# ruchikachavhan/diffusion-models-moe

Hardware: AMD Instinct MI355X
Metric: images/sec SD-1.4 512² 50-step DDIM, expert mask on; 1→8 GPU scaling (higher is better)
Workload: dtype fp16; 1 GPU; SD-1.4 MoE-fied (relu, top-k 0.2, expert 20) + RemoveExperts skilled-expert mask, 512^2 (4x64x64 latents), 50 DDIM steps, CFG 7.5; prompts_per_gpu=8, global_batch=8, parallelism=dp1

## Files before the change

diffusion-models-moe_amd/csrc/gemm.hip:

```cpp
#include <array>
#include <utility>

#include "tune.h"
#include "../../include/sdmoe.h"
#include "gemm_kernel.h"

namespace {

enum TileId { T128x160, T64x160, T256x320, T256x160_42, T256x320_42, T128x320, T128x160_42, T64x320, T128x32, T128x64,
              T128x128, T64x128, NTILE };
struct TileShape { int bm, bn, wmw, wnw; };
constexpr TileShape kTile[NTILE] = {{128, 160, 2, 2}, {64, 160, 2, 2}, {256, 320, 2, 4}, {256, 160, 4, 2},
                                    {256, 320, 4, 2}, {128, 320, 2, 4}, {128, 160, 4, 2}, {64, 320, 2, 4},
                                    {128, 32, 2, 2},  {128, 64, 2, 2},  {128, 128, 2, 2}, {64, 128, 2, 2}};
struct Plan {
  int mode;
  int tile;
  int bk, stages;
  int ksplit;
  int kchunk;
  int kchunk2;
  int mfast;
};
struct TileRule { int tile, ks_want, stages_want; };

constexpr bool built(int mode, int tile) {
  if (mode_halo(mode)) return (tile == T128x320 && mode != MODE_CONVHUP64) || (tile == T256x320 && mode != MODE_CONVHUP16);
  if (mode_geglu(mode))
    return tile == T128x160 || tile == T64x160 || tile == T256x320 || tile == T256x160_42 || tile == T256x320_42 ||
           (tile == T128x160_42 && mode != MODE_GEGLU_GT);
  if (tile == T128x160_42 || tile == T64x320) return mode == MODE_GEMM || mode == MODE_CONV || mode == MODE_GEMM_LN;
  if (tile == T128x32) return mode == MODE_CONV;
  return true;
}
constexpr bool fits3(const TileShape& t, int mode) {
  return GemmLayout{t.bm, t.bn, t.wmw, t.wnw, mode, 3, 64}.SMEM <= 160 * 1024;
}

int device_cus() {
  static int cus = 0;
  int dev = 0, n = 0;
  if (!cus && hipGetDevice(&dev) == hipSuccess &&
// ... 22 lines not shown
    if (ksplit > nk / 4) ksplit = nk / 4;
  }
  while (ksplit > 1 && (long)ksplit * p.M * p.N > ws_floats) --ksplit;
  if (ksplit < 1) ksplit = 1;
  const int kchunk = (nk + ksplit - 1) / ksplit;
  return (nk + kchunk - 1) / kchunk;
}

Plan tile_plan(int mode, int tile, const GemmParams& p, int ksplit, int stages_want) {
  const TileShape& t = kTile[tile];
  const int ntiles = ((p.M + t.bm - 1) / t.bm) * ((p.N + t.bn - 1) / t.bn);
  const int nk = p.K / 64;
  Plan pl{};
  pl.mode = mode; pl.tile = tile; pl.bk = 64; pl.ksplit = ksplit;
  pl.kchunk = (nk + ksplit - 1) / ksplit;
  pl.mfast = (pl.ksplit > 1 && knob(KNOB_MFAST) && (mode == MODE_CONV || mode == MODE_CONV_UP)) ? 1 : 0;
  const int stages = knob(KNOB_STAGES) ? knob(KNOB_STAGES)
                                       : (stages_want ? stages_want : ((t.wmw * t.wnw == 4 && ntiles * pl.ksplit >= 300) ? 2 : 3));
  pl.stages = (stages == 2 || !fits3(t, mode)) ? 2 : 3;
  return pl;
}


Plan halo_plan(int tile, int mode, const GemmParams& p, bool ws, long ws_floats) {
  const int cus = device_cus();
  const int ntiles = (p.M / kTile[tile].bm) * (p.N / 320);
  const int nsl = p.Cin / 32;
  int ksplit = 1;
  const int forced = knob(KNOB_KSPLIT);
  if (ws && forced > 0) {
    ksplit = forced < nsl ? forced : nsl;
// ... 145 lines not shown
  return plan_launch(p.upsample ? MODE_CONV_UP : MODE_CONV, p, ws, ws_floats);
}

template <int MODE, int TILE>
int launch_kernel(const Plan& pl, const GemmParams& p, dim3 grid, hipStream_t s) {
  constexpr TileShape t = kTile[TILE];
  constexpr int NTH = 64 * t.wmw * t.wnw;
  if constexpr (!built(MODE, TILE)) return SDMOE_EUNSUP;
  else if constexpr (mode_halo(MODE)) gemm_kernel<t.bm, t.bn, t.wmw, t.wnw, MODE, 4, 32><<<grid, NTH, 0, s>>>(p);
  else if constexpr (!fits3(t, MODE)) gemm_kernel<t.bm, t.bn, t.wmw, t.wnw, MODE, 2, 64><<<grid, NTH, 0, s>>>(p);
  else if (pl.stages == 2) gemm_kernel<t.bm, t.bn, t.wmw, t.wnw, MODE, 2, 64><<<grid, NTH, 0, s>>>(p);
  else gemm_kernel<t.bm, t.bn, t.wmw, t.wnw, MODE, 3, 64><<<grid, NTH, 0, s>>>(p);
  return SDMOE_OK;
}

constexpr int NMODE = MODE_GEGLU_GT + 1;
using LaunchFn = int (*)(const Plan&, const GemmParams&, dim3, hipStream_t);
template <int... KEY>
constexpr std::array<LaunchFn, sizeof...(KEY)> launch_table(std::integer_sequence<int, KEY...>) {
  return {{&launch_kernel<KEY / NTILE, KEY % NTILE>...}};
}
constexpr auto kLaunch = launch_table(std::make_integer_sequence<int, NMODE * NTILE>{});

int launch(const Plan& pl, GemmParams p, float* ws, hipStream_t s) {
  const TileShape& t = kTile[pl.tile];
  if (p.w_bstride && p.rows_per_batch % t.bm) return SDMOE_EUNSUP;
  if (p.image_set && p.rows_per_batch % t.bm) return SDMOE_EUNSUP;
  if (pl.ksplit > 1 && !ws) return SDMOE_EARG;
  p.ksplit = pl.ksplit; p.kchunk = pl.kchunk; p.kchunk2 = pl.kchunk2; p.mfast = pl.mfast;
  p.part = pl.ksplit > 1 ? ws : nullptr;
  p.diag = knob(KNOB_DIAG); p.res16 = knob(KNOB_RES16);
  const int direct = knob(KNOB_EPI_DIRECT);
  p.epi_direct = direct == 2 || (direct == 1 && p.R == nullptr);
  const dim3 grid(((p.M + t.bm - 1) / t.bm) * ((p.N + t.bn - 1) / t.bn) * pl.ksplit);
  if (const int st = kLaunch[pl.mode * NTILE + pl.tile](pl, p, grid, s)) return st;
  SDMOE_CHECK_LAUNCH();
  if (pl.ksplit > 1) {
    long nchunk = (long)p.M * (p.N / 8);
    int g = (int)((nchunk + 255) / 256);
    if (g > 2048) g = 2048;
    splitk_reduce_kernel<<<g, 256, 0, s>>>(p);
    SDMOE_CHECK_LAUNCH();
  }
  return SDMOE_OK;
}



__global__ __launch_bounds__(256) void gn_apply_kernel(const half_t* __restrict__ X, long ldx, int HW, int C,
                                                       const float* __restrict__ scale, const float* __restrict__ shift,
                                                       int silu, half_t* __restrict__ Y, long ldy, long rows) {
  const int cpr = C / 8;
  const long n = rows * cpr;
  for (long id = blockIdx.x * 256L + threadIdx.x; id < n; id += (long)gridDim.x * 256) {
    const long r = id / cpr;
    const int c = (int)(id - r * cpr) * 8;
// ... 397 lines not shown

extern "C" int sdmoe_conv3x3(const void* X, long ldx, int nimg, int H, int W, int Cin,
                             const void* Wt, const void* bias, const void* coladd, long coladd_bstride,
                             const void* R, long ldr, void* Y, long ldy, int Cout, int stride, int upsample,
                             int act, float* workspace, long workspace_floats, void* stream) {
  if (nimg == 0) return SDMOE_OK;
  if (!X || !Wt || !Y || nimg < 0 || H <= 0 || W <= 0 || Cout <= 0) return SDMOE_EARG;
  if (Cin % 64 || Cout % 8 || ldx % 8 || ldy % 8 || (R && ldr % 8)) return SDMOE_ESHAPE;
  if (!(stride == 1 || stride == 2) || (upsample && stride != 1)) return SDMOE_EUNSUP;
  GemmParams p{};
  conv_shape(p, nimg, H, W, Cin, 0, Cout, stride, upsample, act);
  if (const int st = fill_conv(p, X, ldx, Wt, bias, coladd, coladd_bstride, R, ldr, nullptr, 0, Y, ldy)) return st;
  return launch(plan_conv(p, workspace, workspace_floats), p, workspace, (hipStream_t)stream);
}

extern "C" int sdmoe_conv3x3_sc(const void* X, long ldx, int nimg, int H, int W, int Cin, const void* Wt,
                                const void* bias, const void* coladd, long coladd_bstride, const void* X2, long ldx2,
                                int Cin2, void* Y, long ldy, int Cout, int act, float* workspace,
                                long workspace_floats, void* stream) {
  if (nimg == 0) return SDMOE_OK;
  if (!X || !Wt || !X2 || !Y || nimg < 0 || H <= 0 || W <= 0 || Cout <= 0 || Cin2 <= 0) return SDMOE_EARG;
  if (Cin % 64 || Cin2 % 64 || Cout % 8 || ldx % 8 || ldx2 % 8 || ldy % 8) return SDMOE_ESHAPE;
  GemmParams p{};
  conv_shape(p, nimg, H, W, Cin, Cin2, Cout, 1, 0, act);
  if (const int st = fill_conv(p, X, ldx, Wt, bias, coladd, coladd_bstride, nullptr, 0, X2, ldx2, Y, ldy)) return st;
  return launch(plan_conv(p, workspace, workspace_floats), p, workspace, (hipStream_t)stream);
}

extern "C" int sdmoe_conv3x3_gn(const void* X, long ldx, int nimg, int H, int W, int Cin, const float* gn_scale,
                                const float* gn_shift, int silu, const void* Wt, const void* bias, const void* coladd,
// ... 46 lines not shown
```

diffusion-models-moe_amd/csrc/gemm_kernel.h:

```cpp
#pragma once
#include <type_traits>
#include <utility>
#include "common.h"

namespace {

typedef __attribute__((address_space(3))) void lds_void_t;

struct GemmParams {
  const half_t* A; long lda;
  const half_t* W; long ldw;
  const half_t* bias;
  const half_t* coladd; long coladd_bstride;
  const half_t* R; long ldr;
  half_t* C; long ldc;
  float* part;
  int M, N, K;
  int act;
  int rows_per_batch;
  int H, Wd, Cin, OH, OW, stride, upsample;
  int ksplit, kchunk;
  int kchunk2;
  int mfast;
  int a_bytes, w_bytes;
// ... 78 lines not shown
      for (int j = 0; j < 8; ++j) v[j] += (float)rr[j];
    }
  }
  half8 o;
#pragma unroll
  for (int j = 0; j < 8; ++j) o[j] = (half_t)v[j];
  if (p.diag & 8) {
    asm volatile("" ::"v"(o));
    return;
  }
  *reinterpret_cast<half8*>(p.C + (long)m * p.ldc + n) = o;
}

enum { MODE_GEMM = 0, MODE_CONV = 1, MODE_CONV_UP = 2, MODE_GEGLU = 3, MODE_KEEP = 4, MODE_WMASK = 5, MODE_KEEPW = 6,
       MODE_GEMM_LN = 7, MODE_GEGLU_LN = 8, MODE_CONVH64 = 9, MODE_CONVH32 = 10, MODE_CONVH16 = 11,
       MODE_CONVHUP64 = 12, MODE_CONVHUP32 = 13, MODE_CONVHUP16 = 14, MODE_GEGLU_GT = 15 };
constexpr bool mode_halo(int mode) { return mode >= MODE_CONVH64 && mode <= MODE_CONVHUP16; }
constexpr bool mode_halo_up(int mode) { return mode >= MODE_CONVHUP64 && mode <= MODE_CONVHUP16; }
constexpr int halo_w(int mode) {
  return (mode == MODE_CONVH64 || mode == MODE_CONVHUP64) ? 64 : ((mode == MODE_CONVH32 || mode == MODE_CONVHUP32) ? 32 : 16);
}
constexpr bool mode_akeep(int mode) { return mode == MODE_KEEP || mode == MODE_KEEPW; }
constexpr bool mode_wmask(int mode) { return mode == MODE_WMASK || mode == MODE_KEEPW; }
constexpr bool mode_geglu(int mode) { return mode == MODE_GEGLU || mode == MODE_GEGLU_LN || mode == MODE_GEGLU_GT; }
constexpr bool mode_ln(int mode) { return mode == MODE_GEMM_LN || mode == MODE_GEGLU_LN; }

constexpr int keep_a_bytes(int bm, int mode) { return mode_akeep(mode) ? ((bm * 8 + 1023) / 1024) * 1024 : 0; }
constexpr int keep_w_bytes(int bn, int mode) { return mode_wmask(mode) ? ((bn * 8 + 1023) / 1024) * 1024 : 0; }
constexpr int keep_stage_bytes(int bm, int bn, int mode) { return keep_a_bytes(bm, mode) + keep_w_bytes(bn, mode); }
constexpr int keep_lut_bytes(int mode) { return mode == MODE_KEEP ? 256 * 16 : 16 * 8; }

// ... 30 lines not shown
  int EPI = NW * (WM / NPASS) * WN_PAD * 4, EPI16 = NW * (WM / NPASS16) * RS16 * 2;
  int SMEM0 = (RINGX > EPI) ? (RINGX > EPI16 ? RINGX : EPI16) : (EPI > EPI16 ? EPI : EPI16);
  int LUT_OFF = SMEM0;
  int SMEM1 = SMEM0 + (keep ? keep_lut_bytes(mode) : 0);
  int LN_ROW_OFF = SMEM1, LN_COL_OFF = SMEM1 + bm * 8, LN_IPL = ln ? (bm * 8) / NT : 1;
  int SMEM = SMEM1 + (ln ? bm * 8 + bn * 8 : 0);
  int G_STAGING = NW * 2 * (16 * (FM % 2 == 0 ? 2 : 1)) * (WN / 2) * 2 + NW * WN * 4;
  bool TAB_PREFETCH = mode == MODE_GEGLU_GT && STAGE >= TAB_BYTES && G_STAGING <= STAGE;
  int TAB_LATE_OFF = ((G_STAGING + 1023) / 1024) * 1024;
  bool TAB_OK = mode == MODE_GEGLU_GT && (TAB_PREFETCH || TAB_LATE_OFF + TAB_BYTES <= SMEM1);
};

template <int BM_, int BN_, int WMW_, int WNW_, int MODE_, int NSTAGE_, int BKT_>
struct GemmCfg {
  static constexpr int BM = BM_, BN = BN_, WMW = WMW_, WNW = WNW_, MODE = MODE_, NSTAGE = NSTAGE_, BK = BKT_;
  static constexpr bool CONV = MODE == MODE_CONV || MODE == MODE_CONV_UP, GEGLU = mode_geglu(MODE), LN = mode_ln(MODE);
  static constexpr bool AKEEP = mode_akeep(MODE), WKEEP = mode_wmask(MODE), KEEP = AKEEP || WKEEP;
  static constexpr bool HALO = mode_halo(MODE), HUP = mode_halo_up(MODE);
  static constexpr GemmLayout lay() { return GemmLayout{BM, BN, WMW, WNW, MODE, NSTAGE, BK}; }
  static constexpr int swzk(int row) { return (row >> 1) & (BK / 8 - 1); }
};

SDMOE_DEV float add_f16_lo(float acc, unsigned x) {
  asm("v_fma_mix_f32 %0, %1, 1.0, %0 op_sel_hi:[1,0,0]" : "+v"(acc) : "v"(x));
  return acc;
}
SDMOE_DEV float add_f16_hi(float acc, unsigned x) {
  asm("v_fma_mix_f32 %0, %1, 1.0, %0 op_sel:[1,0,0] op_sel_hi:[1,0,0]" : "+v"(acc) : "v"(x));
  return acc;
}

// ... 49 lines not shown
    tm = bid % ntm;
    const int r = bid / ntm;
    tn = r % ntn;
    split = r / ntn;
  } else {
    split = bid % p.ksplit;
    const int tile = bid / p.ksplit;
    tn = tile % ntn;
    tm = tile / ntn;
  }
  const int m0 = tm * BM, n0 = tn * BN;
  const int nk_total = p.K / BK;
  const int ks0 = split * p.kchunk;
  const int ks1 = min(nk_total, ks0 + p.kchunk);
  const int nk = ks1 - ks0;

  const __amdgpu_buffer_rsrc_t rsA = __builtin_amdgcn_make_buffer_rsrc((void*)p.A, (short)0, p.a_bytes, 0x00020000);
  const half_t* Wimg = p.w_bstride ? p.W + (long)(m0 / p.rows_per_batch) * p.w_bstride : p.W;
  const __amdgpu_buffer_rsrc_t rsW = __builtin_amdgcn_make_buffer_rsrc((void*)Wimg, (short)0, p.w_bytes, 0x00020000);
  const int lrow = lane / L.CPRW, lch = lane % L.CPRW;
  unsigned avoff[L.A_PW];
  unsigned amask[L.A_PW];
  int aoh[L.A_PW], aow[L.A_PW], ab_[L.A_PW];
  unsigned avoff2[L.A_PW];
  unsigned bvoff[L.B_PW];
#pragma unroll
  for (int j = 0; j < L.A_PW; ++j) {
    const int r = L.RPP * (j * L.NW + wave) + lrow;
    const unsigned chb = (unsigned)((lch ^ G::swzk(r)) * 16);
    const int m = m0 + r;
// ... 4 lines not shown
        avoff[j] = (unsigned)((long)m * p.lda * 2) + chb;
      } else {
        const int hw = p.OH * p.OW;
        const int b = m / hw, rr = m - b * hw;
        const int oh = rr / p.OW, ow = rr - oh * p.OW;
        if (MODE == MODE_CONV) {
          const int ih = oh * p.stride, iw = ow * p.stride;
          avoff[j] = (unsigned)(((long)(b * p.H + ih) * p.Wd + iw) * p.lda * 2) + chb;
          unsigned msk = 0;
#pragma unroll
          for (int t = 0; t < 9; ++t) {
            const int y = ih + t / 3 - 1, x = iw + t % 3 - 1;
            msk |= (y >= 0 && y < p.H && x >= 0 && x < p.Wd) ? (1u << t) : 0u;
          }
          amask[j] = msk;
        } else {
          amask[j] = 1; avoff[j] = chb; aoh[j] = oh; aow[j] = ow; ab_[j] = b;
        }
      }
    }
  }
#pragma unroll
  for (int j = 0; j < L.B_PW; ++j) {
    const int r = L.RPP * (j * L.NW + wave) + lrow;
    const int n = n0 + r;
    bvoff[j] = (j * L.NW + wave < L.B_INS && n < p.N) ? (unsigned)((long)n * p.ldw * 2) + (unsigned)((lch ^ G::swzk(r)) * 16)
                                                  : OOB;
  }
  const int kpiece = G::KEEP && wave < L.K_INS ? wave : 0;
  const bool kpa = G::AKEEP && kpiece < L.KA_INS;
// ... 19 lines not shown
        *reinterpret_cast<uint4v*>(smem + L.LUT_OFF + e * 16) = m;
      }
    } else if (tid < 16) {
      const unsigned lo = ((tid & 1) ? 0xFFFFu : 0u) | ((tid & 2) ? 0xFFFF0000u : 0u);
      const unsigned hi = ((tid & 4) ? 0xFFFFu : 0u) | ((tid & 8) ? 0xFFFF0000u : 0u);
      *reinterpret_cast<uint2v*>(smem + L.LUT_OFF + tid * 8) = (uint2v){lo, hi};
    }
    __syncthreads();
  }
  auto a_dst = [&](int j) { return (j * L.NW + wave < L.A_INS) ? (j * L.NW + wave) * 1024 : L.STAGE_AB; };
  auto b_dst = [&](int j) { return (j * L.NW + wave < L.B_INS) ? BM * BK * 2 + (j * L.NW + wave) * 1024 : L.STAGE_AB; };

  const int csl = G::CONV ? p.Cin / BK : 0;
  const __amdgpu_buffer_rsrc_t rsA2 =
      __builtin_amdgcn_make_buffer_rsrc((void*)p.A2, (short)0, p.A2 ? p.a2_bytes : 0, 0x00020000);
  int st_c = G::CONV ? ks0 / 9 : 0, st_tap = G::CONV ? ks0 - st_c * 9 : 0;
  if (MODE == MODE_CONV && ks0 >= 9 * csl) { st_c = csl + (ks0 - 9 * csl); st_tap = 0; }

  auto issue_stage = [&](int ks, int buf) {
    char* sa = smem + buf * L.STAGE;
    const unsigned kb = (unsigned)(ks * BK * 2);
    if (p.diag & 16) {
    } else if (!G::CONV) {
#pragma unroll
      for (int j = 0; j < L.A_PW; ++j) bld16(rsA, sa + a_dst(j), avoff[j], kb);
    } else if (MODE == MODE_CONV && st_c >= csl) {
      const unsigned c2b = (unsigned)((st_c - csl) * BK * 2);
      ++st_c;
#pragma unroll
      for (int j = 0; j < L.A_PW; ++j) bld16(rsA2, sa + a_dst(j), avoff2[j] == OOB ? OOB : avoff2[j] + c2b, 0);
    } else {
      const int tap = st_tap;
      const int kh = tap >= 6 ? 2 : (tap >= 3 ? 1 : 0);
      const int kw = tap - 3 * kh;
      const int c0b = st_c * BK * 2;
      if (++st_tap == 9) { st_tap = 0; ++st_c; }
      if (MODE == MODE_CONV) {
        const unsigned tapoff = (unsigned)(((kh - 1) * p.Wd + (kw - 1)) * (int)p.lda * 2 + c0b);
#pragma unroll
        for (int j = 0; j < L.A_PW; ++j) {
          const unsigned vo = ((amask[j] >> tap) & 1u) ? avoff[j] + tapoff : OOB;
          bld16(rsA, sa + a_dst(j), vo, 0);
        }
      } else {
#pragma unroll
// ... 483 lines not shown
        const float rstd = rsqrtf(var + p.ln_eps);
        ln_row[2 * row] = rstd;
        ln_row[2 * row + 1] = -mean * rstd;
      }
    }
    for (int c = tid; c < BN; c += L.NT) {
      const bool ok = n0 + c < p.N;
      ln_col[c] = ok ? p.ln_wsum[n0 + c] : 0.f;
      ln_col[BN + c] = ok ? p.ln_bias[n0 + c] : 0.f;
    }
  }
  __syncthreads();
  constexpr int CPR = L.WN / 8;
  if (!G::GEGLU && p.act == ACT_NONE && (!p.R || p.res16 != 0)) {
    half4 b4[L.FN];
#pragma unroll
    for (int j = 0; j < L.FN; ++j) {
      const int n = nw + 16 * j + 4 * fg;
      b4[j] = (!G::LN && p.bias && n < p.N) ? *reinterpret_cast<const half4*>(p.bias + n) : (half4){0, 0, 0, 0};
    }
    if (!G::WKEEP && p.epi_direct) {
      const bool res = p.R != nullptr;
#pragma unroll
      for (int i = 0; i < L.FM; ++i) {
        __builtin_amdgcn_sched_barrier(0);
        const int m = mw + 16 * i + fr;
        const half_t* cap = (p.coladd && m < p.M) ? p.coladd + (long)(m / p.rows_per_batch) * p.coladd_bstride : nullptr;
        const float* cfp = (p.colf && m < p.M) ? p.colf + (long)(m / p.rows_per_batch) * p.colf_bstride : nullptr;
        float a = 0.f, c = 0.f;
        if constexpr (G::LN) {
          const int rl = wr * L.WM + 16 * i + fr;
          a = ln_row[2 * rl];
          c = ln_row[2 * rl + 1];
        }
// ... 26 lines not shown
        };
#pragma unroll
        for (int j = 0; j + 1 < L.FN; j += 2) {
          const uint2v ya = frag16(j), yb = frag16(j + 1);
          const auto s0 = __builtin_amdgcn_permlane16_swap(ya[0], yb[0], false, false);
          const auto s1 = __builtin_amdgcn_permlane16_swap(ya[1], yb[1], false, false);
          const int n = nw + 16 * (j + (fg & 1)) + 8 * (fg >> 1);
          half8 o = __builtin_bit_cast(half8, (uint4v){s0[0], s1[0], s0[1], s1[1]});
          if (m < p.M && n < p.N) {
            if (res) {
              const half8 rr = *reinterpret_cast<const half8*>(p.R + (long)m * p.ldr + n);
#pragma unroll
              for (int r = 0; r < 8; ++r) o[r] = (half_t)((float)o[r] + (float)rr[r]);
            }
            if (p.diag & 8) asm volatile("" ::"v"(o));
            else *reinterpret_cast<half8*>(p.C + (long)m * p.ldc + n) = o;
          }
        }
        if constexpr (L.FN % 2) {
          const int n = nw + 16 * (L.FN - 1) + 4 * fg;
          half4 o = __builtin_bit_cast(half4, frag16(L.FN - 1));
          if (m < p.M && n < p.N) {
            if (res) {
              const half4 rr = *reinterpret_cast<const half4*>(p.R + (long)m * p.ldr + n);
#pragma unroll
              for (int r = 0; r < 4; ++r) o[r] = (half_t)((float)o[r] + (float)rr[r]);
            }
            if (p.diag & 8) asm volatile("" ::"v"(o));
            else *reinterpret_cast<half4*>(p.C + (long)m * p.ldc + n) = o;
          }
        }
      }
      return;
    }
    half_t* st = reinterpret_cast<half_t*>(smem) + wave * (L.WM / L.NPASS16) * L.RS16;
    constexpr int NCH16 = (L.WM / L.NPASS16) * CPR, NIT16 = (NCH16 + 63) / 64;
    const bool res = p.R != nullptr;
#pragma unroll
    for (int h = 0; h < L.NPASS16; ++h) {
      half8 rr[NIT16];
      if (res) {
#pragma unroll
        for (int it = 0; it < NIT16; ++it) {
          const int id = lane + 64 * it;
// ... 45 lines not shown
        }
      }
      wave_sync();
#pragma unroll
      for (int it = 0; it < NIT16; ++it) {
        const int id = lane + 64 * it;
        const int r = id / CPR, c8 = id - r * CPR;
        const int m = mw + h * (L.WM / L.NPASS16) + r, n = nw + c8 * 8;
        if (id >= NCH16 || m >= p.M || n >= p.N) continue;
        half8 o = *reinterpret_cast<const half8*>(st + r * L.RS16 + c8 * 8);
        if (res) {
#pragma unroll
          for (int j = 0; j < 8; ++j) o[j] = (half_t)((float)o[j] + (float)rr[it][j]);
        }
        if (p.diag & 8) asm volatile("" ::"v"(o));
        else *reinterpret_cast<half8*>(p.C + (long)m * p.ldc + n) = o;
      }
      wave_sync();
    }
    return;
  }
  if constexpr (G::GEGLU) {
    int lane_o = lane;
    asm volatile("" : "+v"(lane_o));
    const int fr_e = lane_o & 15, fg_e = lane_o >> 4;
    typedef _Float16 h2 __attribute__((ext_vector_type(2)));
    constexpr int NH = L.WN / 2;
    constexpr int FPP = L.FM % 2 == 0 ? 2 : 1;
    constexpr int RG = 16 * FPP;
    constexpr int GST = L.NW * 2 * RG * NH * 2;
    static_assert(NH % 8 == 0, "whole 16-B product chunks per row");
    static_assert(GST + L.NW * L.WN * 4 <= L.SMEM1, "GEGLU staging and bias must fit in the kernel's LDS");
    static_assert(GST + L.NW * L.WN * 4 == L.G_STAGING, "GEGLU staging size as the layout states it");
    constexpr bool gtab = L.TAB_OK;
    char* const sbase = (L.TAB_PREFETCH && gtab) ? smem + ((nk - 1) % NSTAGE) * L.STAGE : smem;
    const half_t* const tab = reinterpret_cast<const half_t*>(
// ... 109 lines not shown
__global__ __launch_bounds__(256) void splitk_reduce_kernel(GemmParams p) {
  const long nchunk = (long)p.M * (p.N / 8);
  for (long id = blockIdx.x * 256L + threadIdx.x; id < nchunk; id += (long)gridDim.x * 256) {
    const int m = (int)(id / (p.N / 8)), n = (int)(id % (p.N / 8)) * 8;
    float v[8] = {0, 0, 0, 0, 0, 0, 0, 0};
    for (int s = 0; s < p.ksplit; ++s) {
      const float* sp = p.part + ((long)s * p.M + m) * p.N + n;
      float4v a = *reinterpret_cast<const float4v*>(sp), b = *reinterpret_cast<const float4v*>(sp + 4);
      v[0] += a[0]; v[1] += a[1]; v[2] += a[2]; v[3] += a[3];
      v[4] += b[0]; v[5] += b[1]; v[6] += b[2]; v[7] += b[3];
    }
    epilogue8(p, m, n, v);
  }
}

}
```

diffusion-models-moe_amd/sdmoe/_lib.py:

```python
from __future__ import annotations

import ctypes
import os

_HERE = os.path.dirname(os.path.abspath(__file__))
LIB_PATH = os.path.join(_HERE, "libsdmoe_hip.so")

_P = ctypes.c_void_p
_L = ctypes.c_long
_I = ctypes.c_int
_F = ctypes.c_float
_FP = ctypes.POINTER(ctypes.c_float)
_IP = ctypes.POINTER(ctypes.c_int)

SIGNATURES = {
    "sdmoe_linear": [_P, _L, _P, _L, _P, _P, _L, _I, _P, _L, _P, _L, _I, _I, _I, _I, _P, _L, _P],
    "sdmoe_conv3x3": [_P, _L, _I, _I, _I, _I, _P, _P, _P, _L, _P, _L, _P, _L, _I, _I, _I, _I, _P, _L, _P],
    "sdmoe_conv3x3_sc": [_P, _L, _I, _I, _I, _I, _P, _P, _P, _L, _P, _L, _I, _P, _L, _I, _I, _P, _L, _P],
    "sdmoe_conv3x3_gn": [_P, _L, _I, _I, _I, _I, _P, _P, _I, _P, _P, _P, _L, _P, _L, _P, _L, _I, _P, _L, _I, _P, _L,
                         _P],
    "sdmoe_groupnorm_apply": [_P, _L, _I, _I, _I, _P, _P, _I, _P, _L, _P],
    "sdmoe_mask_weight": [_P, _P, _L, _L, _P, _P],
    "sdmoe_groupnorm_stats": [_P, _L, _I, _I, _I, _I, _P, _P, _F, _P, _P, _P, _L, _P],
    "sdmoe_groupnorm": [_P, _L, _I, _I, _I, _I, _P, _P, _F, _I, _P, _L, _P, _P, _P, _L, _P],
    "sdmoe_gn_fold": [_P, _L, _I, _I, _P, _P, _P, _I, _P, _P, _P],
    "sdmoe_linear_per_image": [_P, _L, _P, _L, _L, _P, _L, _I, _P, _L, _P, _L, _I, _I, _I, _P, _L, _P],
    "sdmoe_layernorm": [_P, _L, _P, _L, _I, _I, _P, _P, _F, _P],
    "sdmoe_ln_fold": [_P, _L, _I, _I, _P, _P, _P, _P, _L, _P, _P, _P],
    "sdmoe_linear_ln": [_P, _L, _P, _L, _P, _P, _F, _P, _L, _I, _I, _I, _P],
    "sdmoe_linear_geglu_ln": [_P, _L, _P, _L, _P, _P, _F, _P, _L, _I, _I, _I, _I, _P, _L, _I, _P],
    "sdmoe_attention": [_P, _L, _P, _L, _P, _L, _P, _L, _I, _I, _I, _I, _I, _F, _P],
    "sdmoe_geglu_route": [_P, _L, _I, _I, _I, _I, _I, _P, _P, _P, _P, _P, _L, _P, _L, _P, _P, _P],
    "sdmoe_score_bias": [_P, _L, _I, _I, _P, _P, _L, _P],
    "sdmoe_geglu_route_bias": [_P, _L, _I, _I, _I, _I, _I, _P, _P, _P, _P, _P, _L, _P, _L, _P, _P, _P, _P],
    "sdmoe_linear_geglu": [_P, _L, _P, _L, _P, _P, _L, _I, _I, _I, _I, _P, _L, _I, _P],
# ... 112 lines not shown
```

diffusion-models-moe_amd/sdmoe/ops.py:

```python
from __future__ import annotations

import ctypes
import os

import torch

from . import _lib

ACT_NONE, ACT_SILU, ACT_GELU, ACT_RELU, ACT_QUICK_GELU = 0, 1, 2, 3, 4
ACT_BY_NAME = {"none": ACT_NONE, "silu": ACT_SILU, "gelu": ACT_GELU, "relu": ACT_RELU, "quick_gelu": ACT_QUICK_GELU}


_raw_stream = getattr(torch._C, "_cuda_getCurrentRawStream", None)
_cur_dev = getattr(torch._C, "_cuda_getDevice", None)


def _stream():
    if _raw_stream is not None and _cur_dev is not None:
        return _raw_stream(_cur_dev())
    return torch.cuda.current_stream().cuda_stream


def _ptr(t):
    return None if t is None else t.data_ptr()
# ... 362 lines not shown
def conv3x3_launch(xp, ldx, nimg, H, W, Cin, w, bias, coladd, coladd_bstride, rp, ldr, out, op, ldy, Cout, stride,
                   upsample, act, sc=None):
    lib = _lib.load()
    ws = _workspace(out.device)
    if sc is not None:
        st = lib.sdmoe_conv3x3_sc(xp, ldx, nimg, H, W, Cin, _dev(w, "w"), _ptr(bias), _ptr(coladd), coladd_bstride,
                                  sc[0], sc[1], sc[2], op, ldy, Cout, act, ws.data_ptr(), ws.numel(), _stream())
        _lib.check(st, "sdmoe_conv3x3_sc")
        return out
    st = lib.sdmoe_conv3x3(xp, ldx, nimg, H, W, Cin, _dev(w, "w"), _ptr(bias), _ptr(coladd), coladd_bstride, rp, ldr,
                           op, ldy, Cout, stride, int(bool(upsample)), act, ws.data_ptr(), ws.numel(), _stream())
    _lib.check(st, "sdmoe_conv3x3")
    return out


def groupnorm_stats(x, nimg, HW, gamma, beta, eps, groups=32):
    lib = _lib.load()
    xp, ldx = _rows(x, "x")
    C = x.shape[1]
    scale = torch.empty((nimg, C), dtype=torch.float32, device=x.device)
    shift = torch.empty((nimg, C), dtype=torch.float32, device=x.device)
    ws = _gn_workspace(x.device, nimg * groups * 64 * 2)
    st = lib.sdmoe_groupnorm_stats(xp, ldx, nimg, HW, C, groups, _dev(gamma, "gamma"), _dev(beta, "beta"),
                                   float(eps), scale.data_ptr(), shift.data_ptr(), ws.data_ptr(), ws.numel(),
                                   _stream())
    _lib.check(st, "sdmoe_groupnorm_stats")
    return scale, shift


def groupnorm(x, nimg, HW, gamma, beta, eps, groups=32, silu=False, out=None):
# ... 698 lines not shown
```

diffusion-models-moe_amd/sdmoe/unet.py:

```python
from __future__ import annotations

import os

import torch
import torch.nn as nn
import torch.nn.functional as F

from . import ops
from .config import UNetConfig

CTX_LEN = 77
FUSED_GEGLU = True
FUSED_KEEP = True
FUSED_LN = os.environ.get("SDMOE_FUSED_LN", "1") != "0"
FUSED_LN_FFN = os.environ.get("SDMOE_FUSED_LN_FFN", "0") == "1"
FUSED_SC = os.environ.get("SDMOE_FUSED_SC", "1") != "0"
FUSED_GN = os.environ.get("SDMOE_FUSED_GN", "1") != "0"
GN_FOLD_MIN_HW = 1024
IN_PAD = 64
OUT_PAD = 8


def _buf(t):
    return nn.Parameter(t, requires_grad=False)


class LoRACompatibleLinear(nn.Module):

    def __init__(self, weight, bias=None):
        super().__init__()
        self.weight = _buf(weight)
        self.bias = None if bias is None else _buf(bias)
        self._sdmoe_deferred = 0
# ... 428 lines not shown
        if ops.conv_gn_fusable(H, W, cmid, self.conv2.weight.shape[0]):
            gn2 = self.norm2.stats(h, nimg, HW) + (True,)
        else:
            hn = self.norm2.normalize(h, nimg, HW, True)
        if self.conv_shortcut is not None and FUSED_SC and x.shape[1] % 64 == 0:
            w, b = self._conv2_with_shortcut()
            return ops.conv3x3(hn, nimg, H, W, w, b, shortcut=x, out=out, gn=gn2)
        res = x if self.conv_shortcut is None else self.conv_shortcut.run(x)
        return ops.conv3x3(hn, nimg, H, W, self.conv2.weight, self.conv2.bias, residual=res, out=out, gn=gn2)


class Sampler(nn.Module):
    def __init__(self, conv):
        super().__init__()
        self.conv = conv


class Block(nn.Module):

    def __init__(self, resnets, attentions=None, downsamplers=None, upsamplers=None):
        super().__init__()
        self.resnets = nn.ModuleList(resnets)
        if attentions:
            self.attentions = nn.ModuleList(attentions)
        else:
            self.attentions = None
        if downsamplers:
            self.downsamplers = nn.ModuleList(downsamplers)
        if upsamplers:
            self.upsamplers = nn.ModuleList(upsamplers)
# ... 217 lines not shown
                has_up = hasattr(blk, "upsamplers")
                if not last_in_block:
                    nb, ncp, _ = up_in[idx + 1]
                    dest = nb[:, :ncp]
                elif has_up or i == nblk - 1:
                    dest = new(rows, cout)
                if blk.attentions is not None:
                    r = blk.resnets[j].run(inp, nimg, hh, hh, temb_all, out=new(rows, cout))
                    o = blk.attentions[j].run(r, nimg, hh * hh, ctx2d, out=dest)
                else:
                    o = blk.resnets[j].run(inp, nimg, hh, hh, temb_all, out=dest)
                idx += 1
                if last_in_block:
                    if has_up:
                        nb, ncp, _ = up_in[idx]
                        c = blk.upsamplers[0].conv
                        ops.conv3x3(o, nimg, hh, hh, c.weight, c.bias, upsample=True, out=nb[:, :ncp])
                    else:
                        final = o

        fn = self.conv_norm_out.normalize(final, nimg, H * W, True)
        if out is None:
            out = new(nimg * H * W, OUT_PAD)
        return ops.conv3x3(fn, nimg, H, W, self.conv_out.weight, self.conv_out.bias, out=out)

    def forward(self, sample, timestep, encoder_hidden_states, added_cond_kwargs=None):
        n, c, H, W = sample.shape
        x = torch.zeros((n * H * W, IN_PAD), dtype=torch.float16, device=sample.device)
        x[:, :c] = sample.permute(0, 2, 3, 1).reshape(n * H * W, c).to(torch.float16)
        ctx = encoder_hidden_states.reshape(-1, encoder_hidden_states.shape[-1]).to(torch.float16).contiguous()
        add_hidden = None
        if self.config.addition_embed_type == "text_time":
# ... 4 lines not shown
```

include/sdmoe.h:

```cpp
#ifndef SDMOE_H
#define SDMOE_H

#ifdef __cplusplus
extern "C" {
#endif

#define SDMOE_ACT_NONE 0
#define SDMOE_ACT_SILU 1
#define SDMOE_ACT_GELU 2
#define SDMOE_ACT_RELU 3
#define SDMOE_ACT_QUICK_GELU 4

const char* sdmoe_version(void);

int sdmoe_linear(const void* A, long lda, const void* W, long ldw, const void* bias, const void* coladd,
                 long coladd_bstride, int rows_per_batch, const void* R, long ldr, void* C, long ldc, int M, int N,
                 int K, int act, float* workspace, long workspace_floats, void* stream);

int sdmoe_conv3x3(const void* X, long ldx, int nimg, int H, int W, int Cin, const void* Wt, const void* bias,
                  const void* coladd, long coladd_bstride, const void* R, long ldr, void* Y, long ldy, int Cout,
                  int stride, int upsample, int act, float* workspace, long workspace_floats, void* stream);

int sdmoe_conv3x3_sc(const void* X, long ldx, int nimg, int H, int W, int Cin, const void* Wt, const void* bias,
                     const void* coladd, long coladd_bstride, const void* X2, long ldx2, int Cin2, void* Y, long ldy,
                     int Cout, int act, float* workspace, long workspace_floats, void* stream);

int sdmoe_conv3x3_gn(const void* X, long ldx, int nimg, int H, int W, int Cin, const float* gn_scale,
                     const float* gn_shift, int silu, const void* Wt, const void* bias, const void* coladd,
                     long coladd_bstride, const void* R, long ldr, const void* X2, long ldx2, int Cin2, void* Y,
                     long ldy, int Cout, float* workspace, long workspace_floats, void* stream);
int sdmoe_groupnorm_apply(const void* X, long ldx, int nimg, int HW, int C, const float* scale, const float* shift,
                          int silu, void* Y, long ldy, void* stream);

int sdmoe_mask_weight(const void* W, const void* bits, long N, long K, void* Wm, void* stream);

int sdmoe_groupnorm_stats(const void* X, long ldx, int nimg, int HW, int C, int groups, const void* gamma,
                          const void* beta, float eps, float* scale, float* shift, float* workspace,
                          long workspace_floats, void* stream);

int sdmoe_groupnorm(const void* X, long ldx, int nimg, int HW, int C, int groups, const void* gamma, const void* beta,
                    float eps, int silu, void* Y, long ldy, float* scale, float* shift, float* workspace,
                    long workspace_floats, void* stream);

int sdmoe_gn_fold(const void* W, long ldw, int N, int K, const void* bias, const float* scale, const float* shift,
                  int nimg, void* Wf, float* colbias, void* stream);
// ... 131 lines not shown
```

Baseline: 9.390 images/s.

## Collapse nearest-upsample 3x3 conv into four 2x2 sub-pixel convolutions

Adds an UP2X GEMM mode that folds nearest-neighbour 2x upsampling followed by a 3x3 conv into four phase-specific 2x2 convs. The weights are pre-collapsed and cached, and the epilogue and split-K reduce scatter results to interleaved output pixels. This cuts the K dimension from 9*Cin to 4*Cin per output pixel and avoids reading the upsampled input, removing over half the MACs in the upsampler convs. The cost is a scattered output write pattern and a host-side weight transform that is cached on the weight's version.

```diff
diff --git a/diffusion-models-moe_amd/csrc/gemm.hip b/diffusion-models-moe_amd/csrc/gemm.hip
--- a/diffusion-models-moe_amd/csrc/gemm.hip
+++ b/diffusion-models-moe_amd/csrc/gemm.hip
@@ -26,6 +26,9 @@
 
 constexpr bool built(int mode, int tile) {
   if (mode_halo(mode)) return (tile == T128x320 && mode != MODE_CONVHUP64) || (tile == T256x320 && mode != MODE_CONVHUP16);
+  if (mode == MODE_CONV_UP2X)
+    return tile == T128x160 || tile == T64x160 || tile == T256x320 || tile == T256x160_42 || tile == T128x320 ||
+           tile == T128x64 || tile == T128x128 || tile == T64x128;
   if (mode_geglu(mode))
     return tile == T128x160 || tile == T64x160 || tile == T256x320 || tile == T256x160_42 || tile == T256x320_42 ||
            (tile == T128x160_42 && mode != MODE_GEGLU_GT);
@@ -78,7 +81,7 @@
   Plan pl{};
   pl.mode = mode; pl.tile = tile; pl.bk = 64; pl.ksplit = ksplit;
   pl.kchunk = (nk + ksplit - 1) / ksplit;
-  pl.mfast = (pl.ksplit > 1 && knob(KNOB_MFAST) && (mode == MODE_CONV || mode == MODE_CONV_UP)) ? 1 : 0;
+  pl.mfast = (pl.ksplit > 1 && knob(KNOB_MFAST) && (mode == MODE_CONV || mode == MODE_CONV_UP || mode == MODE_CONV_UP2X)) ? 1 : 0;
   const int stages = knob(KNOB_STAGES) ? knob(KNOB_STAGES)
                                        : (stages_want ? stages_want : ((t.wmw * t.wnw == 4 && ntiles * pl.ksplit >= 300) ? 2 : 3));
   pl.stages = (stages == 2 || !fits3(t, mode)) ? 2 : 3;
@@ -254,7 +257,7 @@
   return SDMOE_OK;
 }
 
-constexpr int NMODE = MODE_GEGLU_GT + 1;
+constexpr int NMODE = MODE_CONV_UP2X + 1;
 using LaunchFn = int (*)(const Plan&, const GemmParams&, dim3, hipStream_t);
 template <int... KEY>
 constexpr std::array<LaunchFn, sizeof...(KEY)> launch_table(std::integer_sequence<int, KEY...>) {
@@ -279,7 +282,8 @@
     long nchunk = (long)p.M * (p.N / 8);
     int g = (int)((nchunk + 255) / 256);
     if (g > 2048) g = 2048;
-    splitk_reduce_kernel<<<g, 256, 0, s>>>(p);
+    if (pl.mode == MODE_CONV_UP2X) splitk_reduce_up2x_kernel<<<g, 256, 0, s>>>(p);
+    else splitk_reduce_kernel<<<g, 256, 0, s>>>(p);
     SDMOE_CHECK_LAUNCH();
   }
   return SDMOE_OK;
@@ -707,6 +711,47 @@
   return launch(plan_conv(p, workspace, workspace_floats), p, workspace, (hipStream_t)stream);
 }
 
+namespace {
+
+void up2x_shape(GemmParams& p, int nimg, int H, int W, int Cin, int Cout) {
+  p.M = nimg * H * W; p.N = 4 * Cout; p.K = 4 * Cin; p.act = ACT_NONE;
+  p.ldw = 4L * Cin; p.rows_per_batch = H * W;
+  p.H = H; p.Wd = W; p.Cin = Cin; p.OH = H; p.OW = W; p.stride = 1; p.upsample = 0;
+}
+
+bool plan_up2x(const GemmParams& p, int Cout, bool ws, long ws_floats, Plan* pl) {
+  *pl = plan_launch(MODE_CONV_UP2X, p, ws, ws_floats);
+  return built(MODE_CONV_UP2X, pl->tile) && Cout % kTile[pl->tile].bn == 0;
+}
+
+}
+
+extern "C" int sdmoe_conv_up2x(const void* X, long ldx, int nimg, int H, int W, int Cin, const void* Wc, const void* bias,
+                               void* Y, long ldy, int Cout, float* workspace, long workspace_floats, void* stream) {
+  if (nimg == 0) return SDMOE_OK;
+  if (!X || !Wc || !Y || nimg < 0 || H <= 0 || W <= 0 || Cin <= 0 || Cout <= 0) return SDMOE_EARG;
+  if (Cin % 64 || Cout % 8 || ldx % 8 || ldy % 8) return SDMOE_ESHAPE;
+  if (4L * nimg * H * W >= (long)OOB) return SDMOE_ESHAPE;
+  GemmParams p{};
+  up2x_shape(p, nimg, H, W, Cin, Cout);
+  Plan pl;
+  if (!plan_up2x(p, Cout, workspace, workspace_floats, &pl)) return SDMOE_EUNSUP;
+  if (const int st = fill_conv(p, X, ldx, Wc, bias, nullptr, 0, nullptr, 0, nullptr, 0, Y, ldy)) return st;
+  return launch(pl, p, workspace, (hipStream_t)stream);
+}
+
+extern "C" int sdmoe_conv_up2x_plan(int nimg, int H, int W, int Cin, int Cout, long workspace_floats, int* out) {
+  if (!out || nimg <= 0 || H <= 0 || W <= 0 || Cin <= 0 || Cout <= 0 || workspace_floats < 0) return SDMOE_EARG;
+  if (Cin % 64 || Cout % 8) return SDMOE_ESHAPE;
+  GemmParams p{};
+  up2x_shape(p, nimg, H, W, Cin, Cout);
+  Plan pl;
+  if (!plan_up2x(p, Cout, workspace_floats > 0, workspace_floats, &pl)) return SDMOE_EUNSUP;
+  const TileShape& t = kTile[pl.tile];
+  out[0] = t.bm; out[1] = t.bn; out[2] = t.wmw; out[3] = t.wnw; out[4] = pl.stages; out[5] = pl.ksplit; out[6] = pl.kchunk;
+  return SDMOE_OK;
+}
+
 extern "C" int sdmoe_conv3x3_sc(const void* X, long ldx, int nimg, int H, int W, int Cin, const void* Wt,
                                 const void* bias, const void* coladd, long coladd_bstride, const void* X2, long ldx2,
                                 int Cin2, void* Y, long ldy, int Cout, int act, float* workspace,
diff --git a/diffusion-models-moe_amd/csrc/gemm_kernel.h b/diffusion-models-moe_amd/csrc/gemm_kernel.h
--- a/diffusion-models-moe_amd/csrc/gemm_kernel.h
+++ b/diffusion-models-moe_amd/csrc/gemm_kernel.h
@@ -116,7 +116,13 @@
 
 enum { MODE_GEMM = 0, MODE_CONV = 1, MODE_CONV_UP = 2, MODE_GEGLU = 3, MODE_KEEP = 4, MODE_WMASK = 5, MODE_KEEPW = 6,
        MODE_GEMM_LN = 7, MODE_GEGLU_LN = 8, MODE_CONVH64 = 9, MODE_CONVH32 = 10, MODE_CONVH16 = 11,
-       MODE_CONVHUP64 = 12, MODE_CONVHUP32 = 13, MODE_CONVHUP16 = 14, MODE_GEGLU_GT = 15 };
+       MODE_CONVHUP64 = 12, MODE_CONVHUP32 = 13, MODE_CONVHUP16 = 14, MODE_GEGLU_GT = 15, MODE_CONV_UP2X = 16 };
+SDMOE_DEV long up2x_out_row(int m, int H, int W, int ph) {
+  const int hw = H * W;
+  const int b = m / hw, rq = m - b * hw;
+  const int r = rq / W, q = rq - r * W;
+  return ((long)(b * 2 * H + 2 * r + (ph >> 1)) * (2 * W) + 2 * q + (ph & 1));
+}
 constexpr bool mode_halo(int mode) { return mode >= MODE_CONVH64 && mode <= MODE_CONVHUP16; }
 constexpr bool mode_halo_up(int mode) { return mode >= MODE_CONVHUP64 && mode <= MODE_CONVHUP16; }
 constexpr int halo_w(int mode) {
@@ -177,7 +183,8 @@
 template <int BM_, int BN_, int WMW_, int WNW_, int MODE_, int NSTAGE_, int BKT_>
 struct GemmCfg {
   static constexpr int BM = BM_, BN = BN_, WMW = WMW_, WNW = WNW_, MODE = MODE_, NSTAGE = NSTAGE_, BK = BKT_;
-  static constexpr bool CONV = MODE == MODE_CONV || MODE == MODE_CONV_UP, GEGLU = mode_geglu(MODE), LN = mode_ln(MODE);
+  static constexpr bool UP2X = MODE == MODE_CONV_UP2X;
+  static constexpr bool CONV = MODE == MODE_CONV || MODE == MODE_CONV_UP || UP2X, GEGLU = mode_geglu(MODE), LN = mode_ln(MODE);
   static constexpr bool AKEEP = mode_akeep(MODE), WKEEP = mode_wmask(MODE), KEEP = AKEEP || WKEEP;
   static constexpr bool HALO = mode_halo(MODE), HUP = mode_halo_up(MODE);
   static constexpr GemmLayout lay() { return GemmLayout{BM, BN, WMW, WNW, MODE, NSTAGE, BK}; }
@@ -257,6 +264,7 @@
   const int ks0 = split * p.kchunk;
   const int ks1 = min(nk_total, ks0 + p.kchunk);
   const int nk = ks1 - ks0;
+  const int up_ph = G::UP2X ? n0 / (p.N >> 2) : 0, up_py = up_ph >> 1, up_px = up_ph & 1;
 
   const __amdgpu_buffer_rsrc_t rsA = __builtin_amdgcn_make_buffer_rsrc((void*)p.A, (short)0, p.a_bytes, 0x00020000);
   const half_t* Wimg = p.w_bstride ? p.W + (long)(m0 / p.rows_per_batch) * p.w_bstride : p.W;
@@ -291,6 +299,15 @@
             msk |= (y >= 0 && y < p.H && x >= 0 && x < p.Wd) ? (1u << t) : 0u;
           }
           amask[j] = msk;
+        } else if (G::UP2X) {
+          avoff[j] = (unsigned)(((long)(b * p.H + oh) * p.Wd + ow) * p.lda * 2) + chb;
+          unsigned msk = 0;
+#pragma unroll
+          for (int t = 0; t < 4; ++t) {
+            const int y = oh + up_py + (t >> 1) - 1, x = ow + up_px + (t & 1) - 1;
+            msk |= (y >= 0 && y < p.H && x >= 0 && x < p.Wd) ? (1u << t) : 0u;
+          }
+          amask[j] = msk;
         } else {
           amask[j] = 1; avoff[j] = chb; aoh[j] = oh; aow[j] = ow; ab_[j] = b;
         }
@@ -340,7 +357,8 @@
   const int csl = G::CONV ? p.Cin / BK : 0;
   const __amdgpu_buffer_rsrc_t rsA2 =
       __builtin_amdgcn_make_buffer_rsrc((void*)p.A2, (short)0, p.A2 ? p.a2_bytes : 0, 0x00020000);
-  int st_c = G::CONV ? ks0 / 9 : 0, st_tap = G::CONV ? ks0 - st_c * 9 : 0;
+  constexpr int NTAP = G::UP2X ? 4 : 9;
+  int st_c = G::CONV ? ks0 / NTAP : 0, st_tap = G::CONV ? ks0 - st_c * NTAP : 0;
   if (MODE == MODE_CONV && ks0 >= 9 * csl) { st_c = csl + (ks0 - 9 * csl); st_tap = 0; }
 
   auto issue_stage = [&](int ks, int buf) {
@@ -355,6 +373,17 @@
       ++st_c;
 #pragma unroll
       for (int j = 0; j < L.A_PW; ++j) bld16(rsA2, sa + a_dst(j), avoff2[j] == OOB ? OOB : avoff2[j] + c2b, 0);
+    } else if constexpr (G::UP2X) {
+      const int tap = st_tap;
+      const int c0b = st_c * BK * 2;
+      if (++st_tap == 4) { st_tap = 0; ++st_c; }
+      const unsigned tapoff =
+          (unsigned)(((up_py + (tap >> 1) - 1) * p.Wd + (up_px + (tap & 1) - 1)) * (int)p.lda * 2 + c0b);
+#pragma unroll
+      for (int j = 0; j < L.A_PW; ++j) {
+        const unsigned vo = ((amask[j] >> tap) & 1u) ? avoff[j] + tapoff : OOB;
+        bld16(rsA, sa + a_dst(j), vo, 0);
+      }
     } else {
       const int tap = st_tap;
       const int kh = tap >= 6 ? 2 : (tap >= 3 ? 1 : 0);
@@ -868,10 +897,15 @@
   constexpr int CPR = L.WN / 8;
   if (!G::GEGLU && p.act == ACT_NONE && (!p.R || p.res16 != 0)) {
     half4 b4[L.FN];
+    const int ncol0 = G::UP2X ? up_ph * (p.N >> 2) : 0;
+    auto c_at = [&](int m, int n) -> half_t* {
+      if constexpr (G::UP2X) return p.C + up2x_out_row(m, p.H, p.Wd, up_ph) * p.ldc + (n - ncol0);
+      else return p.C + (long)m * p.ldc + n;
+    };
 #pragma unroll
     for (int j = 0; j < L.FN; ++j) {
       const int n = nw + 16 * j + 4 * fg;
-      b4[j] = (!G::LN && p.bias && n < p.N) ? *reinterpret_cast<const half4*>(p.bias + n) : (half4){0, 0, 0, 0};
+      b4[j] = (!G::LN && p.bias && n < p.N) ? *reinterpret_cast<const half4*>(p.bias + (n - ncol0)) : (half4){0, 0, 0, 0};
     }
     if (!G::WKEEP && p.epi_direct) {
       const bool res = p.R != nullptr;
@@ -928,7 +962,7 @@
               for (int r = 0; r < 8; ++r) o[r] = (half_t)((float)o[r] + (float)rr[r]);
             }
             if (p.diag & 8) asm volatile("" ::"v"(o));
-            else *reinterpret_cast<half8*>(p.C + (long)m * p.ldc + n) = o;
+            else *reinterpret_cast<half8*>(c_at(m, n)) = o;
           }
         }
         if constexpr (L.FN % 2) {
@@ -941,7 +975,7 @@
               for (int r = 0; r < 4; ++r) o[r] = (half_t)((float)o[r] + (float)rr[r]);
             }
             if (p.diag & 8) asm volatile("" ::"v"(o));
-            else *reinterpret_cast<half4*>(p.C + (long)m * p.ldc + n) = o;
+            else *reinterpret_cast<half4*>(c_at(m, n)) = o;
           }
         }
       }
@@ -1017,12 +1051,13 @@
           for (int j = 0; j < 8; ++j) o[j] = (half_t)((float)o[j] + (float)rr[it][j]);
         }
         if (p.diag & 8) asm volatile("" ::"v"(o));
-        else *reinterpret_cast<half8*>(p.C + (long)m * p.ldc + n) = o;
+        else *reinterpret_cast<half8*>(c_at(m, n)) = o;
       }
       wave_sync();
     }
     return;
   }
+  if constexpr (G::UP2X) return;
   if constexpr (G::GEGLU) {
     int lane_o = lane;
     asm volatile("" : "+v"(lane_o));
@@ -1162,4 +1197,30 @@
   }
 }
 
+__global__ __launch_bounds__(256) void splitk_reduce_up2x_kernel(GemmParams p) {
+  const long nchunk = (long)p.M * (p.N / 8);
+  const int cout = p.N >> 2;
+  for (long id = blockIdx.x * 256L + threadIdx.x; id < nchunk; id += (long)gridDim.x * 256) {
+    const int m = (int)(id / (p.N / 8)), n = (int)(id % (p.N / 8)) * 8;
+    float v[8] = {0, 0, 0, 0, 0, 0, 0, 0};
+    for (int s = 0; s < p.ksplit; ++s) {
+      const float* sp = p.part + ((long)s * p.M + m) * p.N + n;
+      float4v a = *reinterpret_cast<const float4v*>(sp), b = *reinterpret_cast<const float4v*>(sp + 4);
+      v[0] += a[0]; v[1] += a[1]; v[2] += a[2]; v[3] += a[3];
+      v[4] += b[0]; v[5] += b[1]; v[6] += b[2]; v[7] += b[3];
+    }
+    const int ph = n / cout, c = n - ph * cout;
+    if (p.bias) {
+      const half8 bb = *reinterpret_cast<const half8*>(p.bias + c);
+#pragma unroll
+      for (int j = 0; j < 8; ++j) v[j] += (float)bb[j];
+    }
+    half8 o;
+#pragma unroll
+    for (int j = 0; j < 8; ++j) o[j] = (half_t)v[j];
+    if (p.diag & 8) asm volatile("" ::"v"(o));
+    else *reinterpret_cast<half8*>(p.C + up2x_out_row(m, p.H, p.Wd, ph) * p.ldc + c) = o;
+  }
 }
+
+}
diff --git a/diffusion-models-moe_amd/sdmoe/_lib.py b/diffusion-models-moe_amd/sdmoe/_lib.py
--- a/diffusion-models-moe_amd/sdmoe/_lib.py
+++ b/diffusion-models-moe_amd/sdmoe/_lib.py
@@ -19,6 +19,8 @@
     "sdmoe_conv3x3_sc": [_P, _L, _I, _I, _I, _I, _P, _P, _P, _L, _P, _L, _I, _P, _L, _I, _I, _P, _L, _P],
     "sdmoe_conv3x3_gn": [_P, _L, _I, _I, _I, _I, _P, _P, _I, _P, _P, _P, _L, _P, _L, _P, _L, _I, _P, _L, _I, _P, _L,
                          _P],
+    "sdmoe_conv_up2x": [_P, _L, _I, _I, _I, _I, _P, _P, _P, _L, _I, _P, _L, _P],
+    "sdmoe_conv_up2x_plan": [_I, _I, _I, _I, _I, _L, _P],
     "sdmoe_groupnorm_apply": [_P, _L, _I, _I, _I, _P, _P, _I, _P, _L, _P],
     "sdmoe_mask_weight": [_P, _P, _L, _L, _P, _P],
     "sdmoe_groupnorm_stats": [_P, _L, _I, _I, _I, _I, _P, _P, _F, _P, _P, _P, _L, _P],
diff --git a/diffusion-models-moe_amd/sdmoe/ops.py b/diffusion-models-moe_amd/sdmoe/ops.py
--- a/diffusion-models-moe_amd/sdmoe/ops.py
+++ b/diffusion-models-moe_amd/sdmoe/ops.py
@@ -400,6 +400,75 @@
     return out
 
 
+_UP2X_TAPS = (((0,), (1, 2)), ((0, 1), (2,)))
+
+
+def up2x_collapse(w):
+    Cout, kh, kw, Cin = w.shape
+    if (kh, kw) != (3, 3):
+        raise ValueError(f"up2x_collapse: expected [Cout, 3, 3, Cin], got {tuple(w.shape)}")
+    out = w.new_empty((4, Cout, 2, 2, Cin))
+    for py in range(2):
+        for px in range(2):
+            for a in range(2):
+                for c in range(2):
+                    taps = [w[:, i, j] for i in _UP2X_TAPS[py][a] for j in _UP2X_TAPS[px][c]]
+                    out[2 * py + px, :, a, c] = sum(taps[1:], taps[0])
+    return out
+
+
+def conv_up2x_weight(w):
+    Cout, _, _, Cin = w.shape
+    if Cin % 64:
+        raise ValueError(f"conv_up2x_weight: Cin % 64 != 0 in {tuple(w.shape)}")
+    wc = up2x_collapse(w.float()).half()
+    return wc.reshape(4, Cout, 4, Cin // 64, 64).permute(0, 1, 3, 2, 4).reshape(4, Cout, Cin // 64, 2, 2, 64).contiguous()
+
+
+def conv_up2x_plan(nimg, H, W, Cin, Cout, workspace_floats=WS_FLOATS):
+    lib = _lib.load()
+    if not _lib.has(lib, "sdmoe_conv_up2x_plan"):
+        return None
+    out = (ctypes.c_int * 7)()
+    st = lib.sdmoe_conv_up2x_plan(nimg, H, W, Cin, Cout, workspace_floats, out)
+    if st in (-2, -3):
+        return None
+    _lib.check(st, "sdmoe_conv_up2x_plan")
+    return {"tile": (out[0], out[1]), "waves": (out[2], out[3]), "stages": out[4], "ksplit": out[5], "kchunk": out[6]}
+
+
+def conv_up2x(x, nimg, H, W, wc, bias=None, out=None, *, fallback=None):
+    xp, ldx = _rows(x, "x")
+    Cin = x.shape[1]
+    if wc.dim() != 6 or wc.shape[0] != 4 or tuple(wc.shape[2:]) != (Cin // 64, 2, 2, 64) or Cin % 64:
+        raise ValueError(f"conv_up2x: weight {tuple(wc.shape)} is not the [4, Cout, Cin/64, 2, 2, 64] layout for "
+                         f"Cin={Cin} (ops.conv_up2x_weight)")
+    Cout = wc.shape[1]
+    if x.shape[0] != nimg * H * W:
+        raise ValueError("conv_up2x: rows != nimg*H*W")
+    if out is None:
+        out = torch.empty((nimg * 4 * H * W, Cout), dtype=torch.float16, device=x.device)
+    elif out.shape[0] != nimg * 4 * H * W or out.shape[1] != Cout:
+        raise ValueError(f"conv_up2x: out {tuple(out.shape)} is not [{nimg * 4 * H * W}, {Cout}]")
+    op, ldy = _rows(out, "out")
+    if conv_up2x_launch(xp, ldx, nimg, H, W, Cin, wc, bias, out, op, ldy, Cout) is not None:
+        return out
+    if fallback is None:
+        raise _lib.SdmoeError(f"sdmoe_conv_up2x refuses Cout={Cout} at {nimg} x {H} x {W} and no fallback filter was given")
+    return conv3x3(x, nimg, H, W, fallback, bias, upsample=True, out=out)
+
+
+def conv_up2x_launch(xp, ldx, nimg, H, W, Cin, wc, bias, out, op, ldy, Cout):
+    lib = _lib.load()
+    ws = _workspace(out.device)
+    st = lib.sdmoe_conv_up2x(xp, ldx, nimg, H, W, Cin, _dev(wc, "wc"), _ptr(bias), op, ldy, Cout, ws.data_ptr(),
+                             ws.numel(), _stream())
+    if st == -3:
+        return None
+    _lib.check(st, "sdmoe_conv_up2x")
+    return out
+
+
 def groupnorm_stats(x, nimg, HW, gamma, beta, eps, groups=32):
     lib = _lib.load()
     xp, ldx = _rows(x, "x")
diff --git a/diffusion-models-moe_amd/sdmoe/unet.py b/diffusion-models-moe_amd/sdmoe/unet.py
--- a/diffusion-models-moe_amd/sdmoe/unet.py
+++ b/diffusion-models-moe_amd/sdmoe/unet.py
@@ -17,6 +17,7 @@
 FUSED_SC = os.environ.get("SDMOE_FUSED_SC", "1") != "0"
 FUSED_GN = os.environ.get("SDMOE_FUSED_GN", "1") != "0"
 GN_FOLD_MIN_HW = 1024
+UPCONV_COLLAPSE = os.environ.get("SDMOE_UPCONV_COLLAPSE", "1") != "0"
 IN_PAD = 64
 OUT_PAD = 8
 
@@ -475,6 +476,24 @@
     def __init__(self, conv):
         super().__init__()
         self.conv = conv
+        self._up2x_key = None
+        self._up2x_w = None
+
+    def _collapsed_weight(self):
+        w = self.conv.weight
+        key = (w.data_ptr(), w._version)
+        if self._up2x_key != key:
+            Cout, nsl = w.shape[0], w.shape[1]
+            taps_last = w.data.permute(0, 2, 3, 1, 4).reshape(Cout, 3, 3, nsl * 64)
+            self._up2x_w = ops.conv_up2x_weight(taps_last)
+            self._up2x_key = key
+        return self._up2x_w
+
+    def upsample(self, x, nimg, H, W, out):
+        c = self.conv
+        if UPCONV_COLLAPSE and ops.conv_up2x_plan(nimg, H, W, x.shape[1], c.weight.shape[0]) is not None:
+            return ops.conv_up2x(x, nimg, H, W, self._collapsed_weight(), c.bias, out=out, fallback=c.weight)
+        return ops.conv3x3(x, nimg, H, W, c.weight, c.bias, upsample=True, out=out)
 
 
 class Block(nn.Module):
@@ -722,8 +741,7 @@
                 if last_in_block:
                     if has_up:
                         nb, ncp, _ = up_in[idx]
-                        c = blk.upsamplers[0].conv
-                        ops.conv3x3(o, nimg, hh, hh, c.weight, c.bias, upsample=True, out=nb[:, :ncp])
+                        blk.upsamplers[0].upsample(o, nimg, hh, hh, nb[:, :ncp])
                     else:
                         final = o
 
diff --git a/include/sdmoe.h b/include/sdmoe.h
--- a/include/sdmoe.h
+++ b/include/sdmoe.h
@@ -29,6 +29,11 @@
                      const float* gn_shift, int silu, const void* Wt, const void* bias, const void* coladd,
                      long coladd_bstride, const void* R, long ldr, const void* X2, long ldx2, int Cin2, void* Y,
                      long ldy, int Cout, float* workspace, long workspace_floats, void* stream);
+
+int sdmoe_conv_up2x(const void* X, long ldx, int nimg, int H, int W, int Cin, const void* Wc, const void* bias, void* Y,
+                    long ldy, int Cout, float* workspace, long workspace_floats, void* stream);
+int sdmoe_conv_up2x_plan(int nimg, int H, int W, int Cin, int Cout, long workspace_floats, int* out);
+
 int sdmoe_groupnorm_apply(const void* X, long ldx, int nimg, int HW, int C, const float* scale, const float* shift,
                           int silu, void* Y, long ldy, void* stream);
 
```

Measured after the change: 9.578 images/s (median of 6 runs). 2.0% higher.
